# liuhatry/xflow

Measured on AMD Instinct MI355X. Metric: samples/sec (whole node) + logloss, LR-FTRL Criteo-1TB shape at 1/2/4/8 MI355X, higher is better.
Workload: dtype fp32; 1 GPU; model=LR-FTRL, global_batch=262144, seq_len=39, parallelism=dp1+table-shard1, rows_per_gpu=262144, nnz_per_row=39, slices=1, grad_layout=unique_lr, hashed_features=1000000000, table_slots_per_gpu=2147483648, backend=hip:gfx950:0, a2a_transport=none, input_overlap=False, table_growths=0

## Files before the change

csrc/engine/engine.cpp:

```cpp
#include <cstdlib>
#include "xflow/engine.h"

#include <algorithm>
#include <atomic>
#include <chrono>
#include <cmath>
#include <cstdio>
#include <cstring>
#include <thread>
#include <fstream>
#include <stdexcept>
#include <string>

namespace xflow {

namespace {

uint64_t next_pow2(uint64_t v) {
  uint64_t p = 1;
  while (p < v) p <<= 1;
  return p;
}

constexpr char kMagic[8] = {'X', 'F', 'L', 'O', 'W', 'T', 'B', '1'};
// ... 460 lines not shown
}

StepInputs Engine::step_inputs() const {
  StepInputs in;
  in.gpu = be_->is_gpu();
  in.remaps = be_->remaps_positions();
  in.red_pairs = red_pairs_ != nullptr;
  in.red_rowv = red_rowv_ != nullptr;
  in.fm_vals = fm_vals_;
  in.csr = cfg_.csr;
  in.sum_slices = cfg_.sum_slices;
  in.kind = cfg_.model.kind;
  in.fm_math = cfg_.model.fm_math;
  in.L = table_.L;
  in.scratch_cap = (double)scratch_.cap;
  in.max_nnz = (double)cfg_.max_nnz;
  in.max_rows = (double)cfg_.max_rows;
  in.pstride = pstride();
  in.slice_cap = slice_cap_;
  in.kdim = cfg_.model.kernel_dim();
  in.lead_handoff = cfg_.lead_handoff;
  in.red_rank = cfg_.red_rank;
  in.red_local = cfg_.red_local;
  return in;
}

StepPlan plan_step(const StepInputs& in, int S) {
  constexpr double k32 = 4294967295.0;
  StepPlan p;
  p.S = S;
  const TableLayout& L = in.L;
  const bool lr16_slot = in.kind == kLR && L.lr16();
  const bool fm_std = in.kind == kFM && in.fm_math == kFmStandard;
  const bool mvm = in.kind == kMVM && in.kdim >= 2;
  const int vnv = fm_std ? 1 + in.kdim : in.kdim;
  const bool std_ok = (fm_std || mvm) && in.gpu && in.red_rowv &&
                      std::ceil(in.max_rows / fmstd_block(vnv - 1)) <= kSegMaxGroups;
  const int csr_min = (in.kind == kLR || fm_std) ? 8 : 4;
  if (in.csr && S >= csr_min && !in.sum_slices && in.red_pairs && in.remaps &&
      (lr16_slot || in.fm_vals || std_ok)) {
    int sl = 0;
    while ((1 << sl) < S) ++sl;
    const int nv = in.fm_vals ? 2 : (std_ok ? vnv : 1);
    if (sl <= red_shift(nv) && in.max_nnz * (double)(1 << sl) < k32) {
      p.csr_slog2 = sl;
      p.csr_rows = std_ok;
// ... 12 lines not shown
                         (in.kind == kLR || in.kind == kFM ||
                          (in.kind == kMVM && in.red_rowv && in.kdim >= 2));
  p.lr16 = lr16_ok && (p.Sf == 1 || (p.masks && red_masks));
  p.lr16s = lr16_ok && p.Sf > 1 && !p.lr16;
  p.uqm = p.masks && red_masks;
  p.fmu = in.fm_vals && (p.Sf == 1 || p.uqm);
  p.fm_keep_w = in.fm_vals && p.groups > 1;
  const bool rows_ok = in.gpu && in.red_pairs && key_bound * in.pstride * in.slice_cap < k32;
  p.mvmu = rows_ok && p.Sf == 1 && in.kind == kMVM && in.red_rowv && in.kdim >= 2;
  p.fsu = rows_ok && (p.Sf == 1 || p.uqm) && in.kind == kFM && in.fm_math == kFmStandard;
  p.rowu = p.mvmu || p.fsu;
  p.grpst = in.gpu && L.opt == kFTRL && L.P > 1;
  p.uq = p.Sf > 1 && (p.lr16 || p.fmu || p.fsu);
  p.grad = p.lr16 ? GradPath::kUniqueLR
           : p.fmu ? GradPath::kUniqueFmBC
           : p.rowu ? GradPath::kUniqueRows
           : p.lr16s ? GradPath::kSlotSums
           : GradPath::kSlotRows;
  p.lead = in.lead_handoff && in.gpu && in.kind == kLR && S == 1 && in.red_pairs && !p.upos &&
           in.field_major && in.rows >= kLeadTile && std::fmod(in.rows, (double)kLeadTile) == 0.0 &&
           in.fields >= 1.0 && in.fields <= kLeadMaxFields && in.scratch_cap < 2147483648.0;
  p.red_rank = in.red_rank && in.gpu && S == 1 && in.red_pairs && !p.upos && (p.lr16 || p.fmu);
  p.red_local = in.red_local && p.lead;
  return p;
}

void Engine::train_step_csr(const BatchView& b, int S, int slog2) {
  const int32_t* srows = slice_rows_dev(b, S);
  const bool fm = fm_vals_;
  const bool rows = csr_full_rows();
  const int ew = rows ? csr_row_words(table_.L.P) : 0;
  float* stash = fm || rows ? grp_nz_.ensure(*be_, 2 * (size_t)cfg_.max_nnz * table_.L.P)
                            : lr_nz_.ensure(*be_, 2 * (size_t)cfg_.max_nnz);
  PullArgs pa = begin_fused_step(b, true, true);
  pa.out_nz = stash;
  be_->table_pull(pa);

  csr_forward_backward(b, slog2, srows, true);

  ApplyArgs aa = apply_args(uniq_keys_, uniq_slot_, ws_->n_uniq, b.nnz, S);
  aa.fm_compact = fm;
  aa.nz_stash = stash;
  aa.csr_off = csr_off_;
  aa.csr_cnt = csr_cnt_;
  aa.csr_ent = rows ? static_cast<const void*>(csr_vent_.get()) : red_pairs_.get();
  aa.csr_ew = ew;
// ... 175 lines not shown
  use_worker_set(0);
  const int S = slices_of(b);
  if (S > cfg_.max_slices) throw std::invalid_argument("batch has more slices than max_slices");
  if (cfg_.sum_slices && slice_groups(S) > 1)
    throw std::invalid_argument("sum_slices: at most 32 slices per step (ordered pushes: any count)");
  const StepPlan P = plan(S, b.rows, b.nnz_per_row, !b.row_ptr && b.col_stride > 0 && b.col_stride == b.rows);
  if (P.grad == GradPath::kCsr) {
    train_step_csr(b, S, P.csr_slog2);
    return;
  }
  const int ng = P.groups;
  const int ps = pstride();
  const bool masks = P.masks;
  const int32_t* srows = slice_rows_dev(b, S);
  const bool uqm = P.uqm, fm_keep_w = P.fm_keep_w, uq = P.uq, upos = P.upos;
  const double key_bound = upos ? (double)cfg_.max_nnz : (double)scratch_.cap;
  struct {
    float* buf = nullptr;
    int width = 0;
    bool normalised = false;
    bool pull_zeroes = true;
  } uo;
  const size_t un = (size_t)cfg_.max_nnz;
  if (P.lr16) {
    uo = {lr_grad_.ensure(*be_, un * slice_cap_), 1, true, true};
  } else if (P.fmu) {
    uo = {fm_grad_.ensure(*be_, 2 * un * slice_cap_), 2, true, true};
  } else if (P.rowu) {
    uo = {row_grad_.ensure(*be_, un * ps * (P.fsu ? slice_cap_ : 1)), ps, false,
          !(P.fsu && P.Sf == 1)};
  }
  float* nz = P.lr16 || P.lr16s ? lr_nz_.ensure(*be_, 2 * un)
              : P.grpst         ? grp_nz_.ensure(*be_, 2 * un * table_.L.P)
                                : nullptr;
  if (fm_keep_w) fm_w_.ensure(*be_, un * ps);
  if (uq) lr_mask_.ensure(*be_, un);

  PullArgs pa = begin_fused_step(b, upos || (uo.buf && !P.red_rank), upos, P.lead);
  if (fm_keep_w) pa.out_w = fm_w_;
  pa.out_nz = nz;
  if (uo.buf && uo.pull_zeroes) {
    pa.zero_out = uo.buf;
    pa.zero_width = uo.width;
  }
  if (uq) {
    pa.zero_out = reinterpret_cast<float*>(lr_mask_.get());
    pa.zero_width = 1;
  }
  be_->table_pull(pa);

  for (int k = 0; k < ng; ++k) {
    const u32* posk = ws_->pos;
    const BatchView bk = group_view(b, S, k, posk);
    const int Sg = group_slices(S, k);
    const int32_t* srk = srows + (int64_t)k * kSliceGroup;
    const bool stash = k == 0;

    FwdArgs fa = train_fwd_args(bk, posk, Sg);
    fa.agg_ok = key_bound * Sg * ps < 4294967295.0;
    if (upos) fa.red_nuq = ws_->n_uniq;
    fa.lead = P.lead;
    fa.red_local = P.red_local;
    if (uq) fa.red_masks = lr_mask_;
    else if (uqm) fa.red_masks = tmask_;
    else if (masks) be_->slice_masks(bk, posk, tmask_);
    fa.fm_compact = fa.red_pairs && fa.agg_ok && cfg_.model.kind == kFM &&
                    cfg_.model.fm_math == kFmReference;
    if (fm_vals_ && !fa.fm_compact) throw std::logic_error("train_step: compact FM rows need the reduction");
    if (uo.buf) {
      fa.red_out = uo.buf;
      fa.red_inv = upos || P.red_rank ? nullptr : ws_->inv.get();
      if (P.red_rank) {
        fa.red_rank_offs = block_counts_;
        fa.red_rank_stamps = scratch_.stamps;
        fa.red_rank_epoch = scratch_.epoch;
      }
      if (uo.normalised) fa.red_rows = srk;
    }
    be_->forward_backward(fa);

    ApplyArgs aa = apply_args(uniq_keys_, uniq_slot_, ws_->n_uniq, b.nnz, Sg);
    aa.sum_slices = cfg_.sum_slices;
    aa.fm_compact = fa.fm_compact;
    if (fm_keep_w) aa.pulled = fm_w_;
    aa.nz_stash = stash ? nz : nullptr;
    if (uo.buf) {
      aa.grads = uo.buf;
      aa.gstride = uo.width;
      aa.slice_rows = uo.normalised ? nullptr : srk;
    } else {
      aa.grads = grad_;
      aa.grad_map = upos ? nullptr : ws_->uniq_pos.get();
      aa.zero_after = true;
      aa.slice_rows = srk;
    }
    if (uq) {
      aa.masks = lr_mask_;
      aa.masks_clear = k + 1 < ng;
    } else if (masks) {
      aa.masks = tmask_;
      aa.masks_rw = tmask_;
    }
// ... 331 lines not shown
                  [&](ApplyArgs& aa, int64_t off, int64_t cnt) {
                    if (off + cnt > sb.n) throw std::invalid_argument("s_apply: offsets beyond pull");
                    aa.grads = base.grads + off * (int64_t)S * gw;
                    if (recv_masks) aa.masks = recv_masks + off;
                  });
}

const float* Engine::pulled_weights(int buf, int64_t off) const {
  const SrvBuf& sb = srv_[buf];
  if (!fm_vals_) return sb.vals + off * (int64_t)pstride();
  if (sb.w_valid) return sb.w + off * (int64_t)pstride();
  return nullptr;
}

void Engine::w_finish() { end_step(); }


bool Engine::snap_ready(int64_t seq) const {
  const volatile unsigned long long* p = &snaps_[seq % kSnaps].word;
  const unsigned long long want = (unsigned long long)seq & ((1ull << (64 - kSnapSeqShift)) - 1);
  return (*p >> kSnapSeqShift) == want;
}

void Engine::attach_snapshot(ApplyArgs& aa) {
  if (!be_->is_gpu() || monitor_disabled() || aa.n_max <= 0) return;
  const int64_t seq = snap_seq_ + 1;
  if (seq - 1 - snap_seen_ >= kSnaps) poll_snapshots(seq - kSnaps);
  aa.snap = &snaps_[seq % kSnaps];
  aa.snap_mon = mon_;
  aa.snap_seq = (unsigned long long)seq;
  snap_carried_ = true;
}

void Engine::poll_snapshots(int64_t wait_upto) {
  while (snap_seen_ < snap_seq_) {
    const int64_t seq = snap_seen_ + 1;
    const int i = (int)(seq % kSnaps);
    if (!snap_ready(seq)) {
      if (seq > wait_upto) break;
      ++monitor_waits_;
      const auto t0 = std::chrono::steady_clock::now();
      for (int spin = 0; !snap_ready(seq); ++spin) {
        if (spin > 64) std::this_thread::sleep_for(std::chrono::microseconds(20));
        else std::this_thread::yield();
      }
      monitor_wait_s_ += std::chrono::duration<double>(std::chrono::steady_clock::now() - t0).count();
    }
    const unsigned long long w = *reinterpret_cast<volatile unsigned long long*>(&snaps_[i].word);
    const int64_t size = (int64_t)(w & 0xFFFFFFFFull);
    const bool ovf0 = (w >> 32) & 1ull, ovf1 = (w >> 33) & 1ull, bad = (w >> 34) & 1ull;
    known_size_ = size;
    known_adds_ = snap_adds_[i];
    ++snap_seen_;
    if (bad && !ovf0 && !ovf1)
      throw std::runtime_error(
// ... 578 lines not shown
```

csrc/hip/hip_util.h:

```cpp
#pragma once

#include <hip/hip_runtime.h>

#include <cstdio>
#include <cstdlib>
#include <stdexcept>
#include <string>

#include "xflow/backend.h"
#include "xflow/common.h"

#define XF_HIP_CHECK(expr)                                                        \
  do {                                                                            \
    hipError_t _e = (expr);                                                       \
    if (_e != hipSuccess) {                                                       \
      throw std::runtime_error(std::string("HIP error: ") + hipGetErrorString(_e) + \
                               " at " __FILE__ ":" + std::to_string(__LINE__) +   \
                               " (" #expr ")");                                   \
    }                                                                             \
  } while (0)

#if defined(XFLOW_DEVICE_ASSERT) && XFLOW_DEVICE_ASSERT
#define XF_DASSERT(cond)                                                           \
  do {                                                                             \
    if (!(cond)) {                                                                 \
      printf("xflow device assert failed: %s at %s:%d\n", #cond, __FILE__, __LINE__); \
      __builtin_trap();                                                            \
    }                                                                              \
  } while (0)
#else
#define XF_DASSERT(cond) \
  do {                   \
  } while (0)
#endif

namespace xflow {
namespace hip {

constexpr int kWave = 64;
constexpr int kBlock = 256;
constexpr int kMaxGrid = 2048;

inline int grid_for(int64_t n, int block = kBlock, int cap = kMaxGrid) {
  if (n <= 0) return 1;
  int64_t g = (n + block - 1) / block;
  return (int)(g < cap ? g : cap);
}

inline int device_cus() {
  static int cached[64] = {};
  int dev = 0;
  if (hipGetDevice(&dev) != hipSuccess || dev < 0 || dev >= 64) return 256;
  if (!cached[dev]) {
    int v = 0;
    if (hipDeviceGetAttribute(&v, hipDeviceAttributeMultiprocessorCount, dev) != hipSuccess || v <= 0)
      v = 256;
    cached[dev] = v;
  }
  return cached[dev];
}

__device__ __forceinline__ int lane_id() { return __lane_id(); }

template <typename T>
// ... 141 lines not shown
```

csrc/hip/kernels_reduce.hip:

```cpp
#include "model_common.h"

namespace xflow {
namespace hip {

__global__ void __launch_bounds__(kBlock) k_red_scan(u32* __restrict__ hist, int groups,
                                                     u32* __restrict__ tot, RedGeom geom,
                                                     int base) {
  if ((int)blockIdx.x >= geom.active(geom.shift(base), (int)gridDim.x)) return;
  const size_t row = (size_t)blockIdx.x * groups;
  u32 carry = 0;
  for (int c0 = 0; c0 < groups; c0 += kBlock) {
    const int i = c0 + (int)threadIdx.x;
    const u32 v = i < groups ? hist[row + i] : 0u;
    u32 t;
    const u32 ex = block_exclusive_scan<kBlock>(v, &t);
    if (i < groups) hist[row + i] = carry + ex;
    carry += t;
  }
  if (threadIdx.x == 0) tot[blockIdx.x] = carry;
}

template <int NV, bool kSeg = false>
__device__ __forceinline__ void red_sum_unit(u64 lo, u32 beg, u32 end,
                                             const void* __restrict__ sorted, const RedFinal& f,
                                             long long* acc, u32* pbits, u32* cbits, u32* rpre,
                                             u32* rwt, const LeadSegs& sg = LeadSegs{}) {
  using T = typename RedRec<NV>::T;
  constexpr int kShift = red_shift(NV);
  constexpr u32 kR = 1u << kShift;
  constexpr int kFx = FxBits<NV>::kFx;
  static_assert(!kSeg || NV == 1, "segments: LR records");
  if (kSeg ? !sg.any : beg == end) return;
  constexpr u32 kRw = kR / 32;
  constexpr u32 kChunkW = (1u << kCompactChunkLog2) / 32;
  static_assert(kRw <= (u32)kRedBlock && kChunkW == 2 * kWave && kRw % kChunkW == 0,
                "a unit is whole chunks, a chunk two waves of bitmap words");
  const bool rank = f.out && f.rk_offs;
  u32 rk_pre = 0;
  if (rank && threadIdx.x < kRw) {
    const u32 w = threadIdx.x;
    const u64 base = lo + 32ull * w;
    u32 m = 0;
    const u64 cap = (u64)*f.rk_cap;
    if (base < cap) {
      const uint4* sp = reinterpret_cast<const uint4*>(f.rk_stamps + base);
      const uint4 q0 = sp[0], q1 = base + 16 < cap ? sp[1] : make_uint4(0u, 0u, 0u, 0u);
      rk_pre = f.rk_offs[base >> kCompactChunkLog2];
      const u32 sw[8] = {q0.x, q0.y, q0.z, q0.w, q1.x, q1.y, q1.z, q1.w};
      const u32 e = f.rk_epoch & 0xFFu;
#pragma unroll
      for (int j = 0; j < 32; ++j) m |= (u32)(((sw[j >> 2] >> (8 * (j & 3))) & 0xFFu) == e) << j;
    }
    pbits[w] = m;
    const u32 c = (u32)__popc(m);
    u32 incl = c;
    const int lane = (int)(w % kWave);
#pragma unroll
    for (int o = 1; o < kWave; o <<= 1) {
      const u32 t = __shfl_up(incl, o);
      if (lane >= o) incl += t;
// ... 183 lines not shown
                            (float)(fx_to_double<kFx>(acc[2 * l + 1]) / rows));
          } else {
            reinterpret_cast<float2*>(f.out)[o] = make_float2(B, C);
          }
        } else {
          *reinterpret_cast<float2*>(f.grad + dest * f.ps) = make_float2(B, C);
        }
        return;
      }
      const float4* v4 = reinterpret_cast<const float4*>(f.wpull + (dest / S) * f.ps);
      float4* g4 = reinterpret_cast<float4*>(f.grad + dest * f.ps);
      for (int q = 0; q < f.ps / 4; ++q) {
        const float4 v = v4[q];
        float o[4] = {v.x, v.y, v.z, v.w};
#pragma unroll
        for (int e = 0; e < 4; ++e) {
          const int c = 4 * q + e;
          o[e] = c == 0 ? (float)f.D * B : (c <= f.D ? C - o[e] * B : 0.0f);
        }
        g4[q] = make_float4(o[0], o[1], o[2], o[3]);
      }
    }
  };
  if (dense) {
    for (u32 l = threadIdx.x; l < kR; l += kRedBlock)
      emit(l, f.masks && ((pbits[l >> 5] >> (l & 31)) & 1u));
    if (f.masks) {
      const u64 s0 = lo / S, s1 = (lo + kR + S - 1) / S;
      for (u64 slot = s0 + threadIdx.x; slot < s1; slot += kRedBlock) {
        const u32 bits = slot_bits<kR>(pbits, slot, S, lo);
        if (bits) put_mask(slot, bits);
      }
    }
  } else {
#pragma unroll
    for (int q = 0; q < kSp; ++q) {
      const u32 l = lr[q];
      if (l >= kR) continue;
      const u32 bit = 1u << (l & 31);
      if (atomicOr(&cbits[l >> 5], bit) & bit) continue;
      emit(l, true);
      if (f.masks) {
        const u64 slot = (lo + l) / S;
        const u32 bits = slot_bits<kR>(pbits, slot, S, lo);
        if (slot * S + (u64)__ffs(bits) - 1 == lo + l) put_mask(slot, bits);
      }
// ... 13 lines not shown
  __shared__ u32 rpre[kR / 32];
  __shared__ u32 rwt[kR / 32 / kWave];
  const int shift = geom.shift(kShift);
  const u32 act = (u32)geom.active(shift, nb);
  const u32 units = act << (shift - kShift);
  u32 id = blockIdx.x, nbeg = 0, nend = 0;
  if (id < units) {
    nbeg = start[id % act];
    nend = start[id % act + 1];
  }
  for (; id < units; id += gridDim.x) {
    const u32 beg = nbeg, end = nend, b = id % act, sub = id / act;
    const u32 nid = id + gridDim.x;
    if (nid < units) {
      nbeg = start[nid % act];
      nend = start[nid % act + 1];
    }
    const u64 lo = ((u64)b << shift) + ((u64)sub << kShift);
    red_sum_unit<NV>(lo, beg, end, sorted, f, acc, pbits, cbits, rpre, rwt);
    lds_barrier();
  }
}

__global__ void __launch_bounds__(kRedBlock) k_red_sum_local(LeadSegs sg, RedFinal f, RedGeom geom,
                                                             int nb) {
  constexpr int kShift = red_shift(1);
  constexpr u32 kR = 1u << kShift;
  constexpr u32 kWaves = kRedBlock / kWave;
  constexpr u32 kSp = 2 * kRedUnroll;
  __shared__ long long acc[kR];
  __shared__ u32 pbits[kR / 32];
  __shared__ u32 cbits[kR / 32];
  __shared__ u32 rpre[kR / 32];
  __shared__ u32 rwt[kR / 32 / kWave];
  __shared__ u32 s_rows[kWaves];
  const int shift = geom.shift(kShift);
  const u32 act = (u32)geom.active(shift, nb);
  const u32 units = act << (shift - kShift);
  const u32 lane = threadIdx.x % kWave, w = threadIdx.x / kWave;
  const u32 per = (sg.groups + kWaves - 1) / kWaves;
  const u32 gb = w * per, ge = gb + per < sg.groups ? gb + per : sg.groups;
  for (u32 id = blockIdx.x; id < units; id += gridDim.x) {
    const u32 b = id % act, sub = id / act;
    sg.row = sg.hist + (size_t)b * sg.groups;
    u32 rows = 0;
    for (u32 c0 = gb; c0 < ge; c0 += kWave) {
      u32 off, cnt;
      sg.seg(c0 + lane < ge ? sg.row[c0 + lane] : 0u, off, cnt);
// ... 204 lines not shown
          if (d < (u64)kCsrHash) add((u32)d, r);
        }
        lds_barrier();
        for (u32 l = (u32)tid; l < (u32)kCsrHash; l += kCsrBlock) {
          const u32 d = sub + l;
          if ((bits[d >> 5] >> (d & 31)) & 1u) emit(out + rank(d), d, &acc[l * NV]);
        }
        lds_barrier();
      }
    }
    out += total;
  }
}

template <int NV>
static RedFinal red_final(const FwdArgs& a) {
  if (a.red_out && (NV == 2 ? !a.fm_compact : false))
    throw std::runtime_error("red_out: compact rows (reference FM)");
  if (a.red_out && a.S != 1 && !a.red_masks)
    throw std::runtime_error("red_out with several slices needs the slice bits (red_masks)");
  RedFinal f{a.grad, a.wpull, a.S, a.model.pstride(), a.model.v_dim,
             a.red_out, a.red_inv, a.red_rows, NV == 2 && a.fm_compact,
             a.S > 1 ? a.red_masks : nullptr};
  if (a.red_rank_offs && a.red_out) {
    if (a.S != 1 || a.red_nuq || !a.red_rank_stamps || !a.red_bcap)
      throw std::runtime_error("red_rank: one slice, slot positions, the batch's stamps and capacity");
    f.rk_offs = a.red_rank_offs;
    f.rk_stamps = a.red_rank_stamps;
    f.rk_cap = a.red_bcap;
    f.rk_epoch = a.red_rank_epoch;
    f.inv = nullptr;
  }
  return f;
}

template <int NV>
void launch_reduction(const FwdArgs& a, int groups, int rows_per_group, hipStream_t st) {
  if (a.red_local) {
    const BatchView& b = a.batch;
    if (NV != 1 || !a.lead || a.S != 1 || a.red_masks || a.red_nuq || a.red_csr.cnt || b.row_ptr ||
        rows_per_group != kLeadTile || b.nnz_per_row < 1 || b.nnz_per_row > kLeadMaxFields ||
        (int64_t)groups * kLeadTile != b.rows)
      throw std::runtime_error("red_local: the LR leader handoff step only (plan_step)");
    LeadSegs sg;
    sg.pairs = a.red_pairs;
    sg.hist = a.red_hist;
    sg.groups = (u32)groups;
    sg.gcap = (u32)(kLeadTile * b.nnz_per_row);
    const u32 grid = std::min<u32>((u32)(a.red_nb * a.red_nsub), (u32)device_cus());
    hipLaunchKernelGGL(k_red_sum_local, dim3(grid), dim3(kRedBlock), 0, st, sg, red_final<1>(a),
                       red_geom(a), a.red_nb);
    return;
  }
  u32* start = a.red_tot + a.red_nb + 1;
  hipLaunchKernelGGL(k_red_scan, dim3(a.red_nb), dim3(kBlock), 0, st, a.red_hist, groups,
                     a.red_tot, red_geom(a), red_shift(NV));
  hipLaunchKernelGGL(k_red_scatter<NV>, dim3(groups), dim3(kRedBlock), 0, st, a.batch,
                     rows_per_group, static_cast<const void*>(a.red_pairs), a.red_count,
                     a.red_hist, a.red_tot, start, a.red_nb, static_cast<void*>(a.red_sorted),
                     red_geom(a));
  if (a.red_csr.cnt) {
    if (!a.red_nuq || a.red_out || a.S != (1 << a.red_csr.slog2) ||
        a.red_csr.slog2 > red_shift(NV) || (NV == 2 && !a.fm_compact))
      throw std::runtime_error("CSR reduction: unique positions, S = 2^slog2 <= 2^shift, no other outputs");
    hipLaunchKernelGGL(k_red_csr<NV>, dim3(a.red_nb), dim3(kCsrBlock), 0, st,
                       static_cast<const void*>(a.red_sorted), start, a.red_csr, red_geom(a), a.red_nb);
    return;
  }
  const RedFinal f = red_final<NV>(a);
  const u32 grid = std::min<u32>((u32)(a.red_nb * a.red_nsub), (u32)device_cus());
  hipLaunchKernelGGL(k_red_sum<NV>, dim3(grid), dim3(kRedBlock), 0, st,
                     static_cast<const void*>(a.red_sorted), start, f, red_geom(a), a.red_nb);
}
template void launch_reduction<1>(const FwdArgs&, int, int, hipStream_t);
// ... 5 lines not shown
```

csrc/hip/model_common.h:

```cpp
#pragma once
#include <cstdio>
#include <cstdlib>
#include <type_traits>
#include "kernels.h"
#include "hip_util.h"

namespace xflow {
namespace hip {

#ifdef XFLOW_KTIMING
static __device__ unsigned long long g_ktime[16];
#define XF_KT_DECL                  \
  unsigned long long kt_acc_[8] = {}; \
  unsigned long long kt_ = clock64()
#define XF_KT(p)                                  \
  do {                                            \
    const unsigned long long n_ = clock64();      \
    kt_acc_[p] += n_ - kt_;                       \
    kt_ = n_;                                     \
  } while (0)
#define XF_KT_FLUSH()                                                    \
  do {                                                                   \
    if (lane_id() == 0) {                                                \
      for (int p_ = 0; p_ < 8; ++p_) atomicAdd(&g_ktime[p_], kt_acc_[p_]); \
// ... 402 lines not shown
      if (i0 + (u32)q * kRedBlock < n) {
        XF_DASSERT((int)(R::dest(pr[q]) >> kShift) < nb);
        p[q] = atomicAdd(&cur[R::dest(pr[q]) >> kShift], 1u);
      }
#pragma unroll
    for (int q = 0; q < kRedUnroll; ++q)
      if (i0 + (u32)q * kRedBlock < n) dst[p[q]] = pr[q];
  }
}

struct RedFinal {
  float* grad;
  const float* wpull;
  int S, ps, D;
  float* out;
  const u32* inv;
  const int32_t* rows;
  bool compact;
  u32* masks;
  const u32* rk_offs = nullptr;
  const unsigned char* rk_stamps = nullptr;
  const unsigned long long* rk_cap = nullptr;
  u32 rk_epoch = 0;
};

template <u32 kR>
__device__ __forceinline__ u32 slot_bits(const u32* pbits, u64 slot, u64 S, u64 lo) {
  u32 bits = 0;
  for (u64 s = 0; s < S; ++s) {
    const u64 d = slot * S + s;
    if (d >= lo && d < lo + kR && ((pbits[(d - lo) >> 5] >> ((d - lo) & 31)) & 1u))
      bits |= 1u << s;
  }
  return bits;
}

template <u32 kR>
__device__ __forceinline__ void unit_masks(const u32* pbits, u64 lo, u64 S, u32* __restrict__ masks,
                                           const u32* __restrict__ inv) {
  const u64 s0 = lo / S, s1 = (lo + kR + S - 1) / S;
  for (u64 slot = s0 + threadIdx.x; slot < s1; slot += blockDim.x) {
    const u32 bits = slot_bits<kR>(pbits, slot, S, lo);
    if (!bits) continue;
    u64 m = slot;
    if (inv) {
      m = inv[slot];
// ... 69 lines not shown
```

csrc/hip/table_common.h:

```cpp
#pragma once
#include <cstdlib>
#include <cstring>
#include <type_traits>

#include "kernels.h"
#include "hip_util.h"

namespace xflow {
namespace hip {

constexpr u32 kNoSlot = 0xFFFFFFFFu;
constexpr int kGroupGridCap = 8192;

constexpr int kScanBlock = 1024;

__device__ __forceinline__ u32 probe(const TableView& t, u64 key, bool insert, bool& claimed) {
  u64 s = table_home(t, fmix64(key));
  const int stride = t.L.stride;
  for (u64 n = 0; n < t.probe_limit; ++n) {
    u64* kp = reinterpret_cast<u64*>(t.words + s * (u64)stride);
    u64 cur = *kp;
    if (cur == key) return (u32)s;
    if (cur == kEmptyKey) {
      if (!insert) return kNoSlot;
      u64 prev = atomicCAS((unsigned long long*)kp, (unsigned long long)kEmptyKey,
                           (unsigned long long)key);
      if (prev == kEmptyKey) { claimed = true; return (u32)s; }
      if (prev == key) return (u32)s;
    }
    s = table_next(t, s);
  }
  if (insert) *t.overflow = 1u;
  return kNoSlot;
}
// ... 98 lines not shown
```

csrc/include/xflow/backend.h:

```cpp
#pragma once

#include <stddef.h>
#include <stdint.h>

#include <memory>
#include <stdexcept>
#include <string>
#include <vector>

#include "xflow/types.h"

namespace xflow {

constexpr u64 kMaxProbe = 1ull << 16;
constexpr int kMaxSegLog2 = 20;

struct TableView {
  u32* words = nullptr;
  u64 cap = 0;
  TableLayout L;
  unsigned long long* size = nullptr;
  u32* overflow = nullptr;
  u64 probe_limit = 0;
  int seg_log2 = 0;
// ... 94 lines not shown
  u32* red_hist = nullptr;
  u32* red_tot = nullptr;
  u32* red_count = nullptr;
  int red_nb = 0;
  int red_maxb = 0;
  int64_t red_sorted_words = 0;
  const unsigned long long* red_bcap = nullptr;
  uint64_t red_cap = 0;
  const int64_t* red_nuq = nullptr;
  unsigned long long* red_records = nullptr;
  u32* red_vmax = nullptr;
  u32* red_vmax_next = nullptr;
  u32* red_dup = nullptr;
  u32* red_dup_next = nullptr;
  int red_nsub = 1;
  int red_groups = 0;
  u32* red_masks = nullptr;
  float* red_out = nullptr;
  const u32* red_inv = nullptr;
  const int32_t* red_rows = nullptr;
  const u32* red_rank_offs = nullptr;
  const unsigned char* red_rank_stamps = nullptr;
  u32 red_rank_epoch = 0;
  bool fm_compact = false;
  float* red_rowv = nullptr;
  CsrOut red_csr;
  u32* fx_bad = nullptr;
};
constexpr int kRedShift = 14;
constexpr int kRedMaxBuckets = 4096;
constexpr int kCsrVecMinShift = 14;
constexpr int red_shift(int nv) {
  return nv == 1 ? kRedShift : (nv == 2 ? kRedShift - 1 : (nv <= 14 ? 10 : (nv <= 28 ? 9 : 8)));
}
constexpr int fmstd_block(int D) { return D <= 10 ? 512 : (D <= 16 ? 256 : 128); }
constexpr int kSegMaxGroups = 2048;
constexpr int64_t fmstd_lds_at(int D, int slots, int maxb) {
  return (int64_t)slots * 8 * (2 + D) + 2 * fmstd_block(D) + (int64_t)maxb * 4 + 1024;
}
constexpr int fmstd_slots(int D) {
  for (int q = 8; q >= 5; --q)
    if (fmstd_lds_at(D, fmstd_block(D) * q / 4, kRedMaxBuckets) <= 80 * 1024)
      return fmstd_block(D) * q / 4;
  return 2 * fmstd_block(D);
}
constexpr int64_t fmstd_lds(int D, int maxb) { return fmstd_lds_at(D, fmstd_slots(D), maxb); }
// ... 478 lines not shown
```

csrc/include/xflow/engine.h:

```cpp
#pragma once

#include <memory>
#include <string>
#include <vector>

#include "xflow/backend.h"
#include "xflow/device_buffer.h"

namespace xflow {

struct EngineConfig {
  ModelSpec model;
  OptSpec opt;
  int table_log2_cap = 20;
  int64_t max_rows = 1 << 16;
  int64_t max_nnz = 1 << 22;
  int max_slices = 1;
  bool sum_slices = false;
  double scratch_factor = 2.5;
  int device = -1;
  bool table_grow = true;
  double grow_load = 0.8;
  double grow_start = 0.6;
  int max_log2_cap = 0;
  int monitor_lag = 2;
  int owner_group = 0;
  bool csr = true;
  int admit_min_count = 1;
  int admit_log2 = 0;
  bool lead_handoff = true;
  bool scratch_carry = true;
  bool red_rank = true;
  bool red_local = true;
  bool delta_track = false;
  int delta_log2 = 0;
};

struct DeltaStats {
  int log2 = 0;
  int64_t bits_set = 0;
  bool needs_full = false;
};

struct ScratchStats {
  int64_t capacity = 0;
  int64_t occupancy = 0;
  int64_t rebuilds = 0;
  int64_t carried = 0;
};

struct StepInputs {
  bool gpu = false;
  bool remaps = false;
  bool red_pairs = false;
  bool red_rowv = false;
  bool fm_vals = false;
  bool csr = true;
  bool sum_slices = false;
  int kind = kLR;
  int fm_math = kFmReference;
  TableLayout L;
  double scratch_cap = 0.0, max_nnz = 0.0, max_rows = 0.0;
  int pstride = 1, slice_cap = 1;
  int kdim = 1;
  bool lead_handoff = true;
  bool field_major = false;
  double rows = 0.0, fields = 0.0;
  bool red_rank = true;
  bool red_local = true;
};

enum class GradPath : int { kCsr = 0, kUniqueLR, kUniqueFmBC, kUniqueRows, kSlotSums, kSlotRows };
const char* grad_path_name(GradPath g);

struct StepPlan {
  int S = 1, groups = 1, Sf = 1;
  int csr_slog2 = -1;
  bool csr_rows = false;
  GradPath grad = GradPath::kSlotRows;
  bool masks = false;
  bool upos = false;
  bool lr16 = false;
  bool lr16s = false;
  bool uqm = false;
  bool fmu = false;
  bool fm_keep_w = false;
  bool mvmu = false, fsu = false, rowu = false;
  bool grpst = false;
  bool uq = false;
  bool lead = false;
  bool red_rank = false;
  bool red_local = false;
};

StepPlan plan_step(const StepInputs& in, int S);

class Engine {
 public:
  explicit Engine(const EngineConfig& cfg);
  ~Engine();
  Engine(const Engine&) = delete;
  Engine& operator=(const Engine&) = delete;

  const EngineConfig& config() const { return cfg_; }
  Backend& backend() { return *be_; }
  bool is_gpu() const { return be_->is_gpu(); }
  void set_stream(void* s) { be_->set_stream(s); }
  void synchronize() { be_->synchronize(); }

  void train_step(const BatchView& b);
  void eval_step(const BatchView& b, float* pctr);

  void push_host(const std::vector<u64>& keys, const std::vector<float>& grads);
  void prefill(int64_t n, uint64_t seed);
  void download_small(void* host_dst, const void* src, size_t bytes) {
// ... 284 lines not shown
    DeviceBuffer<u32> own_pos;
    DeviceBuffer<u64> own_idx;
    SrcGroups grp;
    uint64_t delta_gen = 0;
  };
  SrvBuf srv_[kSrvBufs];
  void stale_stashes() {
    for (SrvBuf& b : srv_) b.nz_fresh = false;
  }
  void mark_stale_buffer(SrvBuf& sb, const u64* keys, int64_t n) {
    if (!delta_bits_ || sb.delta_gen == delta_gen_ || n <= 0) return;
    delta_mark(keys, nullptr, n < sb.n ? n : sb.n);
    sb.delta_gen = delta_gen_;
  }
  bool lr16_layout() const;

  static constexpr int kSnaps = 64;
  HostBuffer<HostSnap> snaps_;
  int64_t snap_adds_[kSnaps] = {};
  bool snap_carried_ = false;
  bool snap_ready(int64_t seq) const;
  void close_snapshot();
  void attach_snapshot(ApplyArgs& aa);
  int64_t snap_seq_ = 0;
  int64_t snap_seen_ = 0;
  int64_t known_size_ = 0;
  int64_t known_adds_ = 0;
  int64_t queued_adds_ = 0;
  int64_t growths_ = 0, splits_ = 0, monitor_waits_ = 0;
  DeviceBuffer<unsigned long long> pruned_dev_;
  int64_t pruned_keys_ = 0;
  double grow_s_ = 0.0;
  u64 max_segs_ = 0;
  double monitor_wait_s_ = 0.0;
  DeviceBuffer<float> grp_nz_;
  DeviceBuffer<unsigned long long> rec_count_;
  DeviceBuffer<u32> red_vmax_;
  DeviceBuffer<u32> text_ws_;
  DeviceBuffer<long long> text_counts_;
  DeviceBuffer<u32> shuf_len_;
  mutable int vmax_parity_ = 0;
  bool rec_on_ = false;
  int log2_cap_ = 0, max_log2_cap_ = 31;
  void poll_snapshots(int64_t wait_upto);
  void guard_inserts(int64_t n);
  void remap_server_slots();
// ... 11 lines not shown
```

csrc/python/module.cpp:

```cpp
#include <pybind11/numpy.h>
#include <pybind11/pybind11.h>
#include <pybind11/stl.h>

#include <algorithm>
#include <atomic>
#include <charconv>
#include <cstdint>
#include <cstdio>
#include <cstring>
#include <thread>
#include <vector>
#include <string>

#include "../comm/async_ps.h"
#include "../comm/rccl_comm.h"
#include "../comm/sharded_step.h"
#include "xflow/engine.h"
#include "xflow/reader.h"
#include "xflow/trainer.h"

namespace py = pybind11;
using namespace xflow;

namespace {
// ... 82 lines not shown
  StepInputs in;
  const ModelSpec m = model_from(d["model"].cast<py::dict>());
  const OptSpec o = opt_from(d["opt"].cast<py::dict>());
  in.kind = m.kind;
  in.fm_math = m.fm_math;
  in.L = TableLayout::make(m, o);
  in.pstride = m.pstride();
  auto flag = [&](const char* k, bool def) { return d.contains(k) ? d[k].cast<bool>() : def; };
  in.gpu = flag("gpu", true);
  in.remaps = flag("remaps", in.gpu);
  in.red_pairs = flag("red_pairs", in.gpu);
  in.red_rowv = flag("red_rowv", in.gpu && (m.kind == kMVM || (m.kind == kFM && m.fm_math == kFmStandard)));
  in.fm_vals = flag("fm_vals", in.gpu && m.kind == kFM && m.fm_math == kFmReference);
  in.csr = flag("csr", true);
  in.sum_slices = flag("sum_slices", false);
  in.max_nnz = d.contains("max_nnz") ? d["max_nnz"].cast<double>() : (double)(1 << 22);
  in.scratch_cap = d.contains("scratch_cap") ? d["scratch_cap"].cast<double>() : 4.0 * in.max_nnz;
  in.slice_cap = d.contains("slice_cap") ? d["slice_cap"].cast<int>() : Engine::kSliceGroup;
  in.max_rows = d.contains("max_rows") ? d["max_rows"].cast<double>() : (double)(1 << 16);
  in.kdim = m.kernel_dim();
  in.lead_handoff = flag("lead_handoff", true);
  in.red_rank = flag("red_rank", true);
  in.red_local = flag("red_local", true);
  in.field_major = flag("field_major", false);
  in.rows = d.contains("rows") ? d["rows"].cast<double>() : 0.0;
  in.fields = d.contains("fields") ? d["fields"].cast<double>() : 0.0;
  return in;
}

}

PYBIND11_MODULE(_xflow_native, m) {
  m.doc() = "xflow-amd native core: HBM hash-table engine, gfx950 kernels, libffm reader";

  m.def("hip_available", &hip_backend_available);
  m.def("plan_step", [](py::dict inputs, int S) { return plan_dict(plan_step(inputs_from(inputs), S)); });
  m.def("write_pred", [](const std::string& path, py::array_t<float> pctr,
                         py::array_t<int32_t> labels) {
    const int64_t n = pctr.size();
    if (labels.size() != n) throw std::invalid_argument("write_pred: lengths differ");
    const float* p = pctr.data();
    const int32_t* y = labels.data();
    py::gil_scoped_release nogil;
    const int64_t per = 1 << 18;
    const int64_t nchunk = (n + per - 1) / per;
    std::vector<std::string> out((size_t)nchunk);
    std::atomic<int64_t> next{0};
    auto work = [&]() {
      for (int64_t c = next++; c < nchunk; c = next++) {
        const int64_t lo = c * per, hi = lo + per < n ? lo + per : n;
        std::string& b = out[(size_t)c];
        b.resize((size_t)(hi - lo) * 24);
        char* q = &b[0];
        for (int64_t i = lo; i < hi; ++i) {
          q = std::to_chars(q, q + 16, (double)p[i], std::chars_format::general, 6).ptr;
          const int yi = y[i] ? 1 : 0;
          *q++ = '\t';
          *q++ = (char)('0' + (1 - yi));
          *q++ = '\t';
// ... 207 lines not shown
      .def("log", [](const AsyncPS& a) { return to_np(a.log()); })
      .def_property_readonly("serving", &AsyncPS::serving)
      .def_property_readonly("transport", &AsyncPS::transport)
      .def_property_readonly("csr", &AsyncPS::csr)
      .def_readonly("steps", &AsyncPS::steps)
      .def_readonly("evals", &AsyncPS::evals)
      .def_readwrite("bytes_moved", &AsyncPS::bytes_moved)
      .def_readwrite("max_staleness", &AsyncPS::max_staleness)
      .def_readwrite("max_lead", &AsyncPS::max_lead)
      .def_readwrite("wait_slot_s", &AsyncPS::wait_slot_s)
      .def_readwrite("wait_pull_s", &AsyncPS::wait_pull_s)
      .def_readwrite("sync_s", &AsyncPS::sync_s)
      .def_readonly("served_pulls", &AsyncPS::served_pulls)
      .def_readonly("applied_pushes", &AsyncPS::applied_pushes)
      .def_readonly("server_busy_s", &AsyncPS::server_busy_s);

  py::class_<Engine>(m, "Engine")
      .def(py::init([](py::dict model, py::dict opt, int table_log2_cap, int64_t max_rows,
                       int64_t max_nnz, int max_slices, bool sum_slices, double scratch_factor,
                       int device, bool table_grow, double grow_load, int max_log2_cap,
                       int monitor_lag, int owner_group, double grow_start, bool csr,
                       int admit_min_count, int admit_log2, bool lead_handoff,
                       bool scratch_carry, bool red_rank, bool delta_track, int delta_log2,
                       bool red_local) {
             EngineConfig c;
             c.red_local = red_local;
             c.delta_track = delta_track;
             c.delta_log2 = delta_log2;
             c.red_rank = red_rank;
             c.lead_handoff = lead_handoff;
             c.scratch_carry = scratch_carry;
             c.admit_min_count = admit_min_count;
             c.admit_log2 = admit_log2;
             c.owner_group = owner_group;
             c.csr = csr;
             c.table_grow = table_grow;
             c.grow_load = grow_load;
             c.grow_start = grow_start;
             c.max_log2_cap = max_log2_cap;
             c.monitor_lag = monitor_lag;
             c.model = model_from(model);
             c.opt = opt_from(opt);
             c.table_log2_cap = table_log2_cap;
             c.max_rows = max_rows;
             c.max_nnz = max_nnz;
             c.max_slices = max_slices;
             c.sum_slices = sum_slices;
             c.scratch_factor = scratch_factor;
             c.device = device;
             return new Engine(c);
           }),
           py::arg("model"), py::arg("opt"), py::arg("table_log2_cap") = 20,
           py::arg("max_rows") = 1 << 16, py::arg("max_nnz") = 1 << 22,
           py::arg("max_slices") = 1, py::arg("sum_slices") = false,
           py::arg("scratch_factor") = 2.5, py::arg("device") = -1,
           py::arg("table_grow") = true, py::arg("grow_load") = 0.8, py::arg("max_log2_cap") = 0,
           py::arg("monitor_lag") = 2, py::arg("owner_group") = 0, py::arg("grow_start") = 0.6,
           py::arg("csr") = true, py::arg("admit_min_count") = 1, py::arg("admit_log2") = 0,
           py::arg("lead_handoff") = true, py::arg("scratch_carry") = true,
           py::arg("red_rank") = true, py::arg("delta_track") = false,
           py::arg("delta_log2") = 0, py::arg("red_local") = true)
      .def("delta_count", &Engine::delta_count, py::call_guard<py::gil_scoped_release>())
      .def("delta_export",
           [](Engine& e) {
             std::vector<u64> k;
             std::vector<u32> w;
             {
               py::gil_scoped_release nogil;
               e.delta_export(k, w);
             }
             return py::make_tuple(to_np(k), to_np(w));
           })
      .def("save_delta", &Engine::save_delta, py::call_guard<py::gil_scoped_release>())
      .def_property_readonly("delta_log2", &Engine::delta_log2)
      .def_property_readonly("delta_needs_full", &Engine::delta_needs_full)
      .def("delta_clear", &Engine::delta_clear, py::call_guard<py::gil_scoped_release>())
      .def("delta_stats",
           [](Engine& e) {
             DeltaStats s;
             {
               py::gil_scoped_release nogil;
               s = e.delta_stats();
             }
             py::dict d;
// ... 16 lines not shown
             {
               py::gil_scoped_release nogil;
               e.admit_export(p);
             }
             return a;
           })
      .def("admit_import",
           [](Engine& e, py::array_t<uint8_t, py::array::c_style | py::array::forcecast> a) {
             if ((size_t)a.size() != e.admit_bytes())
               throw std::invalid_argument("admit_import: size mismatch");
             const uint8_t* p = a.data();
             py::gil_scoped_release nogil;
             e.admit_import(p);
           })
      .def("server_slots", [](Engine& e, int buf) { return to_np(e.server_slots(buf)); },
           py::arg("buf") = 0)
      .def_property_readonly("table_growths", &Engine::table_growths)
      .def_property_readonly("csr_steps", &Engine::csr_steps)
      .def("step_plan",
           [](const Engine& e, int S, int64_t rows, int64_t fields, bool field_major) {
             const StepPlan p = e.plan(S, rows, fields, field_major);
             py::dict d = plan_dict(p);
             d["red_local"] = p.red_local;
             return d;
           },
           py::arg("S"), py::arg("rows") = 0, py::arg("fields") = 0, py::arg("field_major") = false)
      .def_property_readonly("table_splits", &Engine::table_splits)
      .def_property_readonly("table_geometry", &Engine::table_geometry)
      .def_property_readonly("table_committed", &Engine::table_committed)
      .def_property_readonly("grow_seconds", &Engine::grow_seconds)
      .def_property_readonly("monitor_waits", &Engine::monitor_waits)
      .def_property_readonly("monitor_wait_seconds", &Engine::monitor_wait_seconds)
      .def("parse_text",
           [](Engine& e, uintptr_t text, int64_t n, uintptr_t keys, uintptr_t fgid,
              uintptr_t row_ptr, uintptr_t labels, int64_t max_rows, int64_t max_nnz,
              int64_t row_mod) {
             return e.parse_text(P<const char>(text), n, P<u64>(keys), P<int32_t>(fgid),
                                 P<int32_t>(row_ptr), P<float>(labels), max_rows, max_nnz,
                                 row_mod);
           },
           py::arg("text"), py::arg("n"), py::arg("keys"), py::arg("fgid"), py::arg("row_ptr"),
           py::arg("labels"), py::arg("max_rows"), py::arg("max_nnz"), py::arg("row_mod") = 1,
           py::call_guard<py::gil_scoped_release>())
      .def("count_records", &Engine::count_records)
      .def("take_records", &Engine::take_records, py::call_guard<py::gil_scoped_release>())
      .def("grow_table", &Engine::grow_table, py::call_guard<py::gil_scoped_release>())
// ... 449 lines not shown
```

xflow_amd/config.py:

```python
from __future__ import annotations

import dataclasses
import os
from dataclasses import dataclass, field

MODEL_KINDS = {"lr": 0, "fm": 1, "mvm": 2}
MODEL_NAMES = {v: k for k, v in MODEL_KINDS.items()}
OPT_KINDS = {"ftrl": 0, "sgd": 1}
FM_MATH = {"reference": 0, "standard": 1}
MVM_MATH = {"compat": 0, "fixed": 1}


def model_kind(m) -> int:
    if isinstance(m, int):
        if m not in MODEL_NAMES:
            raise ValueError(f"model index must be 0 (LR), 1 (FM) or 2 (MVM), got {m}")
        return m
    m = str(m).lower()
    if m in ("0", "1", "2"):
        return int(m)
    if m not in MODEL_KINDS:
        raise ValueError(f"unknown model {m!r}; expected lr/fm/mvm")
    return MODEL_KINDS[m]

# ... 72 lines not shown


@dataclass
class EngineConfig:
    table_log2_cap: int = 22
    max_rows: int = 1 << 16
    max_nnz: int = 1 << 22
    max_slices: int = 1
    sum_slices: bool = False
    scratch_factor: float = 2.5
    table_grow: bool = True
    grow_load: float = 0.8
    grow_start: float = 0.6
    max_log2_cap: int = 0
    monitor_lag: int = 2
    owner_group: int = 0
    csr: bool = True
    admit_min_count: int = 1
    admit_log2: int = 0
    lead_handoff: bool = True
    scratch_carry: bool = True
    red_rank: bool = True
    red_local: bool = True
    delta_track: bool = False
    delta_log2: int = 0


@dataclass
class TrainConfig:
    train_prefix: str = ""
    test_prefix: str = ""
    epochs: int = 60
    threads: int = 0
    train_block_bytes: int = 2 << 20
    block_rows: int = 0
    fixed_width: bool = True
    resident: bool = False
    shuffle: bool = False
    shuffle_seed: int = 0
    copy_threads: int = 8
    gpu_parse: bool = False
    test_block_bytes: int = 0
    serial_slices: bool = False
    keep_remainder: bool = False
    mvm_predict_compat: bool = False
    init_push: bool = True
# ... 31 lines not shown
```

xflow_amd/engine.py:

```python
from __future__ import annotations

from dataclasses import dataclass
from typing import Optional

import numpy as np
import torch

from xflow_amd import native
from xflow_amd.config import EngineConfig, ModelConfig, OptimConfig, check_crosses


@dataclass
class Batch:

    keys: torch.Tensor
    labels: torch.Tensor
    row_ptr: Optional[torch.Tensor] = None
    fgid: Optional[torch.Tensor] = None
    nnz_per_row: int = 0
    slice_rows: int = 0
    field_major: bool = False

    @property
    def rows(self) -> int:
# ... 129 lines not shown
        self.model = model or ModelConfig()
        self.optim = optim or OptimConfig()
        self.cfg = engine or EngineConfig()
        self.device = torch.device(device)
        if self.device.type == "cuda":
            native.require_hip()
            if self.device.index is None:
                self.device = torch.device("cuda", torch.cuda.current_device())
        n = native.load()
        self._e = n.Engine(self.model.native(), self.optim.native(),
                           table_log2_cap=self.cfg.table_log2_cap, max_rows=self.cfg.max_rows,
                           max_nnz=self.cfg.max_nnz, max_slices=self.cfg.max_slices,
                           sum_slices=self.cfg.sum_slices, scratch_factor=self.cfg.scratch_factor,
                           device=_device_index(self.device), table_grow=self.cfg.table_grow,
                           grow_load=self.cfg.grow_load, max_log2_cap=self.cfg.max_log2_cap,
                           monitor_lag=self.cfg.monitor_lag, owner_group=self.cfg.owner_group,
                           grow_start=self.cfg.grow_start, csr=self.cfg.csr,
                           admit_min_count=self.cfg.admit_min_count,
                           admit_log2=self.cfg.admit_log2,
                           lead_handoff=self.cfg.lead_handoff,
                           scratch_carry=self.cfg.scratch_carry,
                           red_rank=self.cfg.red_rank,
                           red_local=self.cfg.red_local,
                           delta_track=self.cfg.delta_track,
                           delta_log2=self.cfg.delta_log2)
        if self.is_gpu != (self.device.type == "cuda"):
            raise RuntimeError("native engine backend does not match the requested device")

    @property
    def native(self):
        return self._e

    @property
    def is_gpu(self) -> bool:
        return bool(self._e.is_gpu)

    @property
    def backend_name(self) -> str:
        return self._e.backend_name

    @property
    def pstride(self) -> int:
        return int(self._e.pstride)

    @property
    def grad_width(self) -> int:
# ... 451 lines not shown
```

Measured before the change: 769.0 million samples/s.

## Fuse FTRL apply into the ranked local reduction kernel for LR

Adds a red_apply path, on by default, for the ranked, bucket-local LR step: the reduction kernel normalises each unique key's summed gradient, then applies the FTRL update and writes z/n straight to the table slots. The separate gradient buffer write, its zeroing and the separate apply kernel launch are skipped. The host snapshot store moves into the reduction kernel. The cost is a longer, more complex reduce kernel with extra LDS traffic and scattered global table writes inside it.

```diff
diff --git a/csrc/engine/engine.cpp b/csrc/engine/engine.cpp
--- a/csrc/engine/engine.cpp
+++ b/csrc/engine/engine.cpp
@@ -506,6 +506,7 @@
   in.lead_handoff = cfg_.lead_handoff;
   in.red_rank = cfg_.red_rank;
   in.red_local = cfg_.red_local;
+  in.red_apply = cfg_.red_apply;
   return in;
 }
 
@@ -564,6 +565,7 @@
            in.fields >= 1.0 && in.fields <= kLeadMaxFields && in.scratch_cap < 2147483648.0;
   p.red_rank = in.red_rank && in.gpu && S == 1 && in.red_pairs && !p.upos && (p.lr16 || p.fmu);
   p.red_local = in.red_local && p.lead;
+  p.red_apply = in.red_apply && p.red_local && p.red_rank && p.lr16;
   return p;
 }
 
@@ -785,7 +787,9 @@
     bool pull_zeroes = true;
   } uo;
   const size_t un = (size_t)cfg_.max_nnz;
-  if (P.lr16) {
+  if (P.red_apply) {
+    uo = {nullptr, 1, true, false};
+  } else if (P.lr16) {
     uo = {lr_grad_.ensure(*be_, un * slice_cap_), 1, true, true};
   } else if (P.fmu) {
     uo = {fm_grad_.ensure(*be_, 2 * un * slice_cap_), 2, true, true};
@@ -830,7 +834,7 @@
     fa.fm_compact = fa.red_pairs && fa.agg_ok && cfg_.model.kind == kFM &&
                     cfg_.model.fm_math == kFmReference;
     if (fm_vals_ && !fa.fm_compact) throw std::logic_error("train_step: compact FM rows need the reduction");
-    if (uo.buf) {
+    if (uo.buf || P.red_apply) {
       fa.red_out = uo.buf;
       fa.red_inv = upos || P.red_rank ? nullptr : ws_->inv.get();
       if (P.red_rank) {
@@ -840,7 +844,15 @@
       }
       if (uo.normalised) fa.red_rows = srk;
     }
+    if (P.red_apply) {
+      fa.red_apply_words = table_.words;
+      fa.red_apply_slots = uniq_slot_;
+      fa.red_apply_nz = nz;
+      fa.red_apply_ftrl = cfg_.opt.ftrl;
+      attach_snapshot(fa, b.nnz);
+    }
     be_->forward_backward(fa);
+    if (P.red_apply) continue;
 
     ApplyArgs aa = apply_args(uniq_keys_, uniq_slot_, ws_->n_uniq, b.nnz, Sg);
     aa.sum_slices = cfg_.sum_slices;
@@ -1218,15 +1230,18 @@
   return (*p >> kSnapSeqShift) == want;
 }
 
-void Engine::attach_snapshot(ApplyArgs& aa) {
-  if (!be_->is_gpu() || monitor_disabled() || aa.n_max <= 0) return;
+template <typename Args>
+void Engine::attach_snapshot_to(Args& a, int64_t n_max) {
+  if (!be_->is_gpu() || monitor_disabled() || n_max <= 0) return;
   const int64_t seq = snap_seq_ + 1;
   if (seq - 1 - snap_seen_ >= kSnaps) poll_snapshots(seq - kSnaps);
-  aa.snap = &snaps_[seq % kSnaps];
-  aa.snap_mon = mon_;
-  aa.snap_seq = (unsigned long long)seq;
+  a.snap = &snaps_[seq % kSnaps];
+  a.snap_mon = mon_;
+  a.snap_seq = (unsigned long long)seq;
   snap_carried_ = true;
 }
+void Engine::attach_snapshot(ApplyArgs& aa) { attach_snapshot_to(aa, aa.n_max); }
+void Engine::attach_snapshot(FwdArgs& fa, int64_t n_max) { attach_snapshot_to(fa, n_max); }
 
 void Engine::poll_snapshots(int64_t wait_upto) {
   while (snap_seen_ < snap_seq_) {
diff --git a/csrc/hip/hip_util.h b/csrc/hip/hip_util.h
--- a/csrc/hip/hip_util.h
+++ b/csrc/hip/hip_util.h
@@ -40,6 +40,7 @@
 constexpr int kWave = 64;
 constexpr int kBlock = 256;
 constexpr int kMaxGrid = 2048;
+constexpr u32 kNoSlot = 0xFFFFFFFFu;
 
 inline int grid_for(int64_t n, int block = kBlock, int cap = kMaxGrid) {
   if (n <= 0) return 1;
diff --git a/csrc/hip/kernels_reduce.hip b/csrc/hip/kernels_reduce.hip
--- a/csrc/hip/kernels_reduce.hip
+++ b/csrc/hip/kernels_reduce.hip
@@ -35,7 +35,8 @@
   constexpr u32 kChunkW = (1u << kCompactChunkLog2) / 32;
   static_assert(kRw <= (u32)kRedBlock && kChunkW == 2 * kWave && kRw % kChunkW == 0,
                 "a unit is whole chunks, a chunk two waves of bitmap words");
-  const bool rank = f.out && f.rk_offs;
+  const bool apply = kSeg && f.ap_slots;
+  const bool rank = (f.out || apply) && f.rk_offs;
   u32 rk_pre = 0;
   if (rank && threadIdx.x < kRw) {
     const u32 w = threadIdx.x;
@@ -265,6 +266,70 @@
       }
     }
   };
+  if constexpr (kSeg) {
+    if (apply) {
+      constexpr u32 kNone = 0xFFFFFFFFu;
+      const u32 r0 = rpre[0];
+      u32 cnt = 0;
+#pragma unroll
+      for (u32 i = 0; i < kRw / kWave; ++i) cnt += rwt[i];
+      u32* aw = reinterpret_cast<u32*>(acc);
+      auto put_sum = [&](u32 l) {
+        aw[2 * l] = __float_as_uint((float)(fx_to_double<kFx>(acc[l]) / (double)f.rows[0]));
+      };
+      u32 mine = 0;
+      if (dense) {
+        for (u32 l = threadIdx.x; l < kR; l += kRedBlock)
+          if (rank_of(l) != kNone) put_sum(l);
+      } else {
+#pragma unroll
+        for (int q = 0; q < kSp; ++q) {
+          const u32 l = lr[q];
+          if (l >= kR) continue;
+          const u32 bit = 1u << (l & 31);
+          if (atomicOr(&cbits[l >> 5], bit) & bit) continue;
+          if (rank_of(l) == kNone) continue;
+          mine |= 1u << q;
+          put_sum(l);
+        }
+      }
+      lds_barrier();
+      if (dense) {
+        for (u32 l = threadIdx.x; l < kR; l += kRedBlock) {
+          const u32 o = rank_of(l);
+          if (o != kNone) aw[2 * (o - r0) + 1] = l;
+        }
+      } else {
+#pragma unroll
+        for (int q = 0; q < kSp; ++q)
+          if (mine & (1u << q)) aw[2 * (rank_of(lr[q]) - r0) + 1] = lr[q];
+      }
+      lds_barrier();
+      constexpr int kAp = 4;
+      const FtrlParams fp = f.ap_fp;
+      for (u32 j0 = threadIdx.x; j0 < cnt; j0 += kAp * kRedBlock) {
+        u32 slot[kAp];
+        float2 nz[kAp];
+        float g[kAp];
+#pragma unroll
+        for (int q = 0; q < kAp; ++q) {
+          const u32 j = j0 + (u32)q * kRedBlock;
+          const u32 jc = j < cnt ? j : cnt - 1u;
+          slot[q] = f.ap_slots[r0 + jc];
+          nz[q] = f.ap_nz[r0 + jc];
+          g[q] = __uint_as_float(aw[2 * (aw[2 * jc + 1] & (kR - 1u))]);
+        }
+#pragma unroll
+        for (int q = 0; q < kAp; ++q) {
+          if (j0 + (u32)q * kRedBlock >= cnt || slot[q] == kNoSlot) continue;
+          const float w = ftrl_weight(nz[q].y, nz[q].x, fp);
+          ftrl_push(nz[q].x, nz[q].y, w, g[q], fp);
+          *reinterpret_cast<float2*>(f.ap_words + (u64)slot[q] * 4 + 2) = nz[q];
+        }
+      }
+      return;
+    }
+  }
   if (dense) {
     for (u32 l = threadIdx.x; l < kR; l += kRedBlock)
       emit(l, f.masks && ((pbits[l >> 5] >> (l & 31)) & 1u));
@@ -324,8 +389,14 @@
   }
 }
 
+struct RedSnap {
+  HostSnap* dst = nullptr;
+  const u32* mon = nullptr;
+  unsigned long long seq = 0;
+};
 __global__ void __launch_bounds__(kRedBlock) k_red_sum_local(LeadSegs sg, RedFinal f, RedGeom geom,
-                                                             int nb) {
+                                                             int nb, RedSnap snap) {
+  if (snap.dst) store_snapshot(snap.dst, snap.mon, snap.seq);
   constexpr int kShift = red_shift(1);
   constexpr u32 kR = 1u << kShift;
   constexpr u32 kWaves = kRedBlock / kWave;
@@ -576,7 +647,16 @@
   RedFinal f{a.grad, a.wpull, a.S, a.model.pstride(), a.model.v_dim,
              a.red_out, a.red_inv, a.red_rows, NV == 2 && a.fm_compact,
              a.S > 1 ? a.red_masks : nullptr};
-  if (a.red_rank_offs && a.red_out) {
+  if (a.red_apply_slots) {
+    if (NV != 1 || !a.red_local || a.red_out || !a.red_rank_offs || !a.red_rows ||
+        !a.red_apply_words || !a.red_apply_nz)
+      throw std::runtime_error("red_apply: the ranked bucket-sorted LR step only (plan_step)");
+    f.ap_words = a.red_apply_words;
+    f.ap_slots = a.red_apply_slots;
+    f.ap_nz = reinterpret_cast<const float2*>(a.red_apply_nz);
+    f.ap_fp = a.red_apply_ftrl;
+  }
+  if (a.red_rank_offs && (a.red_out || a.red_apply_slots)) {
     if (a.S != 1 || a.red_nuq || !a.red_rank_stamps || !a.red_bcap)
       throw std::runtime_error("red_rank: one slice, slot positions, the batch's stamps and capacity");
     f.rk_offs = a.red_rank_offs;
@@ -602,8 +682,10 @@
     sg.groups = (u32)groups;
     sg.gcap = (u32)(kLeadTile * b.nnz_per_row);
     const u32 grid = std::min<u32>((u32)(a.red_nb * a.red_nsub), (u32)device_cus());
+    RedSnap snap;
+    if (a.red_apply_slots) snap = {a.snap, a.snap_mon, a.snap_seq};
     hipLaunchKernelGGL(k_red_sum_local, dim3(grid), dim3(kRedBlock), 0, st, sg, red_final<1>(a),
-                       red_geom(a), a.red_nb);
+                       red_geom(a), a.red_nb, snap);
     return;
   }
   u32* start = a.red_tot + a.red_nb + 1;
diff --git a/csrc/hip/model_common.h b/csrc/hip/model_common.h
--- a/csrc/hip/model_common.h
+++ b/csrc/hip/model_common.h
@@ -448,6 +448,10 @@
   const unsigned char* rk_stamps = nullptr;
   const unsigned long long* rk_cap = nullptr;
   u32 rk_epoch = 0;
+  u32* ap_words = nullptr;
+  const u32* ap_slots = nullptr;
+  const float2* ap_nz = nullptr;
+  FtrlParams ap_fp;
 };
 
 template <u32 kR>
diff --git a/csrc/hip/table_common.h b/csrc/hip/table_common.h
--- a/csrc/hip/table_common.h
+++ b/csrc/hip/table_common.h
@@ -9,7 +9,6 @@
 namespace xflow {
 namespace hip {
 
-constexpr u32 kNoSlot = 0xFFFFFFFFu;
 constexpr int kGroupGridCap = 8192;
 
 constexpr int kScanBlock = 1024;
diff --git a/csrc/include/xflow/backend.h b/csrc/include/xflow/backend.h
--- a/csrc/include/xflow/backend.h
+++ b/csrc/include/xflow/backend.h
@@ -140,6 +140,13 @@
   const u32* red_rank_offs = nullptr;
   const unsigned char* red_rank_stamps = nullptr;
   u32 red_rank_epoch = 0;
+  u32* red_apply_words = nullptr;
+  const u32* red_apply_slots = nullptr;
+  const float* red_apply_nz = nullptr;
+  FtrlParams red_apply_ftrl;
+  struct HostSnap* snap = nullptr;
+  const u32* snap_mon = nullptr;
+  unsigned long long snap_seq = 0;
   bool fm_compact = false;
   float* red_rowv = nullptr;
   CsrOut red_csr;
diff --git a/csrc/include/xflow/engine.h b/csrc/include/xflow/engine.h
--- a/csrc/include/xflow/engine.h
+++ b/csrc/include/xflow/engine.h
@@ -32,6 +32,7 @@
   bool scratch_carry = true;
   bool red_rank = true;
   bool red_local = true;
+  bool red_apply = true;
   bool delta_track = false;
   int delta_log2 = 0;
 };
@@ -68,6 +69,7 @@
   double rows = 0.0, fields = 0.0;
   bool red_rank = true;
   bool red_local = true;
+  bool red_apply = true;
 };
 
 enum class GradPath : int { kCsr = 0, kUniqueLR, kUniqueFmBC, kUniqueRows, kSlotSums, kSlotRows };
@@ -91,6 +93,7 @@
   bool lead = false;
   bool red_rank = false;
   bool red_local = false;
+  bool red_apply = false;
 };
 
 StepPlan plan_step(const StepInputs& in, int S);
@@ -421,6 +424,9 @@
   bool snap_ready(int64_t seq) const;
   void close_snapshot();
   void attach_snapshot(ApplyArgs& aa);
+  void attach_snapshot(FwdArgs& fa, int64_t n_max);
+  template <typename Args>
+  void attach_snapshot_to(Args& a, int64_t n_max);
   int64_t snap_seq_ = 0;
   int64_t snap_seen_ = 0;
   int64_t known_size_ = 0;
diff --git a/csrc/python/module.cpp b/csrc/python/module.cpp
--- a/csrc/python/module.cpp
+++ b/csrc/python/module.cpp
@@ -128,6 +128,7 @@
   in.lead_handoff = flag("lead_handoff", true);
   in.red_rank = flag("red_rank", true);
   in.red_local = flag("red_local", true);
+  in.red_apply = flag("red_apply", true);
   in.field_major = flag("field_major", false);
   in.rows = d.contains("rows") ? d["rows"].cast<double>() : 0.0;
   in.fields = d.contains("fields") ? d["fields"].cast<double>() : 0.0;
@@ -140,7 +141,18 @@
   m.doc() = "xflow-amd native core: HBM hash-table engine, gfx950 kernels, libffm reader";
 
   m.def("hip_available", &hip_backend_available);
-  m.def("plan_step", [](py::dict inputs, int S) { return plan_dict(plan_step(inputs_from(inputs), S)); });
+  m.def(
+      "plan_step",
+      [](py::dict inputs, int S, bool batch) {
+        const StepPlan p = plan_step(inputs_from(inputs), S);
+        py::dict d = plan_dict(p);
+        if (batch) {
+          d["red_local"] = p.red_local;
+          d["red_apply"] = p.red_apply;
+        }
+        return d;
+      },
+      py::arg("inputs"), py::arg("S"), py::arg("batch") = false);
   m.def("write_pred", [](const std::string& path, py::array_t<float> pctr,
                          py::array_t<int32_t> labels) {
     const int64_t n = pctr.size();
@@ -394,9 +406,10 @@
                        int monitor_lag, int owner_group, double grow_start, bool csr,
                        int admit_min_count, int admit_log2, bool lead_handoff,
                        bool scratch_carry, bool red_rank, bool delta_track, int delta_log2,
-                       bool red_local) {
+                       bool red_local, bool red_apply) {
              EngineConfig c;
              c.red_local = red_local;
+             c.red_apply = red_apply;
              c.delta_track = delta_track;
              c.delta_log2 = delta_log2;
              c.red_rank = red_rank;
@@ -431,7 +444,8 @@
            py::arg("csr") = true, py::arg("admit_min_count") = 1, py::arg("admit_log2") = 0,
            py::arg("lead_handoff") = true, py::arg("scratch_carry") = true,
            py::arg("red_rank") = true, py::arg("delta_track") = false,
-           py::arg("delta_log2") = 0, py::arg("red_local") = true)
+           py::arg("delta_log2") = 0, py::arg("red_local") = true,
+           py::arg("red_apply") = true)
       .def("delta_count", &Engine::delta_count, py::call_guard<py::gil_scoped_release>())
       .def("delta_export",
            [](Engine& e) {
@@ -494,6 +508,7 @@
              const StepPlan p = e.plan(S, rows, fields, field_major);
              py::dict d = plan_dict(p);
              d["red_local"] = p.red_local;
+             d["red_apply"] = p.red_apply;
              return d;
            },
            py::arg("S"), py::arg("rows") = 0, py::arg("fields") = 0, py::arg("field_major") = false)
diff --git a/xflow_amd/config.py b/xflow_amd/config.py
--- a/xflow_amd/config.py
+++ b/xflow_amd/config.py
@@ -118,6 +118,7 @@
     scratch_carry: bool = True
     red_rank: bool = True
     red_local: bool = True
+    red_apply: bool = True
     delta_track: bool = False
     delta_log2: int = 0
 
diff --git a/xflow_amd/engine.py b/xflow_amd/engine.py
--- a/xflow_amd/engine.py
+++ b/xflow_amd/engine.py
@@ -175,6 +175,7 @@
                            scratch_carry=self.cfg.scratch_carry,
                            red_rank=self.cfg.red_rank,
                            red_local=self.cfg.red_local,
+                           red_apply=self.cfg.red_apply,
                            delta_track=self.cfg.delta_track,
                            delta_log2=self.cfg.delta_log2)
         if self.is_gpu != (self.device.type == "cuda"):
```

Result: faster. 790.5 million samples/s (median of 6 runs) (+2.8%).
